# openxrlab/xrslam

Measured on AMD Instinct MI355X. Metric: frames/sec, full per-frame hot path (KLT tracker + sliding-window VI-BA), one sequence per GPU, higher is better.
Workload: dtype u8/i16 images, f32 LK with exact i64 reductions, f64 BA

## Files before the change

xrslam_amd/csrc/host/geometry.hpp:

```cpp
#pragma once
#include <array>
#include <cmath>
#include <map>
#include <numeric>
#include <random>
#include <vector>

#include "hla.hpp"

namespace xrh {

struct Intrinsics {
    double fx = 1, fy = 1, cx = 0, cy = 0;
};

inline V2 apply_k(V3 p, const Intrinsics &K) { return {p.x / p.z * K.fx + K.cx, p.y / p.z * K.fy + K.cy}; }
inline V3 remove_k(V2 p, const Intrinsics &K) { return normalized(V3{(p.x - K.cx) / K.fx, (p.y - K.cy) / K.fy, 1.0}); }

struct P34 {
    double m[12];
};
inline std::array<double, 4> triangulate_point(const std::vector<P34> &Ps, const std::vector<V3> &zs) {
    Dense A((int)zs.size() * 2, 4);
    for (size_t i = 0; i < zs.size(); ++i)
        for (int c = 0; c < 4; ++c) {
            A((int)i * 2, c) = zs[i].x * Ps[i].m[8 + c] - zs[i].z * Ps[i].m[c];
            A((int)i * 2 + 1, c) = zs[i].y * Ps[i].m[8 + c] - zs[i].z * Ps[i].m[4 + c];
        }
    std::vector<double> s;
    Dense V;
    jacobi_svd(A, s, V);
    return {V(0, 3), V(1, 3), V(2, 3), V(3, 3)};
}

class LotBox {
  public:
    explicit LotBox(size_t size) : cap_(0), lots_(size) { std::iota(lots_.begin(), lots_.end(), 0); }
    void seed(unsigned v) { engine_.seed(v); }
    void refill_all() { cap_ = 0; }
    size_t remaining() const { return lots_.size() - cap_; }
    size_t draw_without_replacement() {
        if (remaining() > 1) {
            std::uniform_int_distribution<size_t>::param_type pr(cap_, lots_.size() - 1);
            std::swap(lots_[cap_], lots_[dist_(engine_, pr)]);
            return lots_[cap_++];
        } else if (remaining() == 1) {
            cap_++;
            return lots_.back();
        }
        return size_t(-1);
    }

  private:
    size_t cap_;
    std::vector<size_t> lots_;
    std::default_random_engine engine_;
    std::uniform_int_distribution<size_t> dist_;
};

namespace fivept {

inline constexpr int pidx(int ex, int ey, int ez) { return ex * 16 + ey * 4 + ez; }
template <int D> struct Sup;
template <> struct Sup<1> {
    static constexpr int N = 4;
    static constexpr unsigned char idx[4] = {0, 1, 4, 16};
};
template <> struct Sup<2> {
    static constexpr int N = 10;
    static constexpr unsigned char idx[10] = {0, 1, 2, 4, 5, 8, 16, 17, 20, 32};
};
template <> struct Sup<3> {
    static constexpr int N = 20;
    static constexpr unsigned char idx[20] = {0, 1, 2, 3, 4, 5, 6, 8, 9, 12, 16, 17, 18, 20, 21, 24, 32, 33, 36, 48};
};
template <int D> inline constexpr int rank_of(int dense) {
    for (int k = 0; k < Sup<D>::N; ++k)
        if (Sup<D>::idx[k] == dense) return k;
    return -1;
}
template <int D> struct Poly {
    double c[Sup<D>::N];
    Poly() {
        for (double &v : c) v = 0.0;
    }
    double at(int ex, int ey, int ez) const { return c[rank_of<D>(pidx(ex, ey, ez))]; }
    double &at(int ex, int ey, int ez) { return c[rank_of<D>(pidx(ex, ey, ez))]; }
};
template <int D> inline Poly<D> padd(const Poly<D> &a, const Poly<D> &b, double sb = 1.0) {
    Poly<D> r;
    for (int k = 0; k < Sup<D>::N; ++k) r.c[k] = a.c[k] + sb * b.c[k];
    return r;
}
template <int D> inline Poly<D> pscale(const Poly<D> &a, double s) {
    Poly<D> r;
    for (int k = 0; k < Sup<D>::N; ++k) r.c[k] = a.c[k] * s;
    return r;
}
template <int DA, int DB> struct MulTable {
    unsigned char t[Sup<DA>::N][Sup<DB>::N];
    constexpr MulTable() : t() {
        for (int p = 0; p < Sup<DA>::N; ++p)
            for (int q = 0; q < Sup<DB>::N; ++q) t[p][q] = (unsigned char)rank_of<DA + DB>(Sup<DA>::idx[p] + Sup<DB>::idx[q]);
    }
};
template <int DA, int DB> inline Poly<DA + DB> pmul(const Poly<DA> &a, const Poly<DB> &b) {
    static constexpr MulTable<DA, DB> T{};
    Poly<DA + DB> r;
    for (int p = 0; p < Sup<DA>::N; ++p) {
        const double av = a.c[p];
        if (av == 0.0) continue;
        for (int q = 0; q < Sup<DB>::N; ++q) {
            const double bv = b.c[q];
            if (bv == 0.0) continue;
            r.c[T.t[p][q]] += av * bv;
        }
    }
    return r;
}

static constexpr int MONO[20][3] = {{3, 0, 0}, {2, 1, 0}, {1, 2, 0}, {0, 3, 0}, {2, 0, 1}, {1, 1, 1}, {0, 2, 1},
                                {1, 0, 2}, {0, 1, 2}, {0, 0, 3}, {2, 0, 0}, {1, 1, 0}, {0, 2, 0}, {1, 0, 1},
                                {0, 1, 1}, {0, 0, 2}, {1, 0, 0}, {0, 1, 0}, {0, 0, 1}, {0, 0, 0}};
enum { XXX = 0, XXY, XYY, YYY, XXZ, XYZ, YYZ, XZZ, YZZ, ZZZ, XX, XY, YY, XZ, YZ, ZZ, X, Y, Z, I };
struct MonoRank {
    unsigned char r[20];
    constexpr MonoRank() : r() {
        for (int m = 0; m < 20; ++m) r[m] = (unsigned char)rank_of<3>(pidx(MONO[m][0], MONO[m][1], MONO[m][2]));
    }
};

}

inline std::vector<M3> solve_essential_5pt(const std::array<V2, 5> &p1, const std::array<V2, 5> &p2) {
    using namespace fivept;
    for (int i = 0; i < 5; ++i)
        if (!std::isfinite(p1[i].x) || !std::isfinite(p1[i].y) || !std::isfinite(p2[i].x) || !std::isfinite(p2[i].y)) return {};
    Dense A(5, 9);
    for (int i = 0; i < 5; ++i) {
        const double h1[3] = {p1[i].x, p1[i].y, 1.0}, h2[3] = {p2[i].x, p2[i].y, 1.0};
        for (int j = 0; j < 3; ++j)
            for (int k = 0; k < 3; ++k) A(i, j * 3 + k) = h1[j] * h2[k];
    }
    std::vector<double> sv;
    Dense V;
    jacobi_svd(A, sv, V);
    double B[4][3][3];
    for (int b = 0; b < 4; ++b)
        for (int col = 0; col < 3; ++col)
            for (int row = 0; row < 3; ++row) B[b][row][col] = V(col * 3 + row, 5 + b);
    Poly<1> E[3][3];
    for (int i = 0; i < 3; ++i)
        for (int j = 0; j < 3; ++j) {
            E[i][j].at(1, 0, 0) = B[0][i][j];
            E[i][j].at(0, 1, 0) = B[1][i][j];
            E[i][j].at(0, 0, 1) = B[2][i][j];
            E[i][j].at(0, 0, 0) = B[3][i][j];
        }
    Poly<2> EEt[3][3];
    for (int i = 0; i < 3; ++i)
        for (int j = 0; j < 3; ++j) {
            Poly<2> s;
            for (int k = 0; k < 3; ++k) s = padd(s, pmul(E[i][k], E[j][k]));
            EEt[i][j] = s;
        }
    const Poly<2> tr = padd(padd(EEt[0][0], EEt[1][1]), EEt[2][2]);
    const Poly<2> half_tr = pscale(tr, 0.5);
    Dense polys(10, 20);
    static constexpr MonoRank MR{};
    for (int i = 0; i < 3; ++i)
        for (int j = 0; j < 3; ++j) {
            Poly<3> s;
            for (int k = 0; k < 3; ++k) s = padd(s, pmul(EEt[i][k], E[k][j]));
            s = padd(s, pmul(half_tr, E[i][j]), -1.0);
            for (int m = 0; m < 20; ++m) polys(i * 3 + j, m) = s.c[MR.r[m]];
        }
    {
        auto minor = [&](int r0, int c0, int r1, int c1, int r2, int c2, int r3, int c3) {
            return padd(pmul(E[r0][c0], E[r1][c1]), pmul(E[r2][c2], E[r3][c3]), -1.0);
        };
        const Poly<3> d = padd(padd(pmul(E[0][0], minor(1, 1, 2, 2, 1, 2, 2, 1)), pmul(E[0][1], minor(1, 0, 2, 2, 1, 2, 2, 0)), -1.0),
                               pmul(E[0][2], minor(1, 0, 2, 1, 1, 1, 2, 0)));
        for (int m = 0; m < 20; ++m) polys(9, m) = d.c[MR.r[m]];
    }
    std::array<int, 10> perm;
    for (int i = 0; i < 10; ++i) perm[i] = i;
    for (int i = 0; i < 10; ++i) {
        for (int j = i + 1; j < 10; ++j)
            if (std::fabs(polys(perm[i], i)) < std::fabs(polys(perm[j], i))) std::swap(perm[i], perm[j]);
        if (polys(perm[i], i) == 0) continue;
        const double d = polys(perm[i], i);
        for (int c = 0; c < 20; ++c) polys(perm[i], c) /= d;
        for (int j = i + 1; j < 10; ++j) {
            const double f = polys(perm[j], i);
            for (int c = 0; c < 20; ++c) polys(perm[j], c) -= polys(perm[i], c) * f;
        }
    }
    for (int i = 9; i > 0; --i)
        for (int j = 0; j < i; ++j) {
            const double f = polys(perm[j], i);
            for (int c = 0; c < 20; ++c) polys(perm[j], c) -= polys(perm[i], c) * f;
        }
    Dense action(10, 10);
    const int rows[6] = {XXX, XXY, XYY, XXZ, XYZ, XZZ};
    for (int r = 0; r < 6; ++r)
        for (int c = 0; c < 10; ++c) action(r, c) = -polys(perm[rows[r]], XX + c);
    action(6, XX - XX) = 1.0;
    action(7, XY - XX) = 1.0;
    action(8, XZ - XX) = 1.0;
    action(9, X - XX) = 1.0;
    std::vector<double> wr, wi;
    std::vector<std::vector<double>> vecs;
    real_eigen(action, wr, wi, vecs);
    std::vector<M3> out;
    for (int e = 0; e < 10; ++e) {
        if (vecs[e].empty()) continue;
        const std::vector<double> &h = vecs[e];
        const double w = h[I - XX];
        const double xs = h[X - XX] / w, ys = h[Y - XX] / w, zs = h[Z - XX] / w;
        M3 Em;
        for (int i = 0; i < 3; ++i)
            for (int j = 0; j < 3; ++j) Em(i, j) = B[0][i][j] * xs + B[1][i][j] * ys + B[2][i][j] * zs + B[3][i][j];
        out.push_back(Em);
    }
    return out;
}

inline double essential_geometric_error(const M3 &E, V2 p1, V2 p2) {
    V3 Ep1 = E * V3{p1.x, p1.y, 1.0};
    double r = p2.x * Ep1.x + p2.y * Ep1.y + Ep1.z;
    return r * r / (Ep1.x * Ep1.x + Ep1.y * Ep1.y);
}

inline M3 solve_rotation_2pt(const std::array<V3, 2> &a, const std::array<V3, 2> &b) {
    Dense cov(3, 3);
    for (int k = 0; k < 2; ++k)
        for (int i = 0; i < 3; ++i)
            for (int j = 0; j < 3; ++j) cov(i, j) += a[k][i] * b[k][j];
    for (double &v : cov.a) v *= 0.5;
    std::vector<double> s;
    Dense V, U;
    jacobi_svd(cov, s, V, &U);
    V3 u0{U(0, 0), U(1, 0), U(2, 0)}, u1{U(0, 1), U(1, 1), U(2, 1)}, u2{U(0, 2), U(1, 2), U(2, 2)};
    if (!(s[2] > 1e-12 * std::max(s[0], 1e-300))) {
        u2 = normalized(cross(u0, u1));
    }
    M3 Um, Vm;
    for (int i = 0; i < 3; ++i) {
        Um(i, 0) = u0[i];
        Um(i, 1) = u1[i];
        Um(i, 2) = u2[i];
        for (int j = 0; j < 3; ++j) Vm(i, j) = V(i, j);
    }
    M3 D = M3::identity();
    D(2, 2) = det(Vm * transpose(Um)) >= 0.0 ? 1.0 : -1.0;
    return Vm * D * transpose(Um);
}

template <size_t DoF, class Sample1, class Sample2, class Solver, class Evaluator>
M3 ransac_solve(const std::vector<Sample1> &d1, const std::vector<Sample2> &d2, double threshold, double confidence,
                size_t max_iteration, int seed, Solver solver, Evaluator make_eval, std::vector<char> &inlier_mask) {
    const size_t size = d1.size();
    LotBox lotbox(size);
    lotbox.seed((unsigned)seed);
    const double K = std::log(std::max(1 - confidence, 1.0e-5));
    size_t inlier_count = 0;
    M3 model;
    if (size < DoF) {
        inlier_mask.assign(size, 0);
        return model;
    }
    size_t iter_max = max_iteration;
    std::vector<char> cur_mask;
    for (size_t iter = 0; iter < iter_max; ++iter) {
        std::array<Sample1, DoF> s1;
        std::array<Sample2, DoF> s2;
        lotbox.refill_all();
        for (size_t si = 0; si < DoF; ++si) {
            size_t idx = lotbox.draw_without_replacement();
            s1[si] = d1[idx];
            s2[si] = d2[idx];
        }
        std::vector<M3> models = solver(s1, s2);
        for (const M3 &cur : models) {
            if (inlier_count == size) break;
            size_t cur_count = 0;
            cur_mask.assign(size, 0);
            auto eval = make_eval(cur);
            for (size_t i = 0; i < size; ++i) {
                double err = eval(d1[i], d2[i]);
                if (err <= threshold) {
                    cur_count++;
                    cur_mask[i] = 1;
                }
            }
            if (cur_count > inlier_count) {
                model = cur;
                inlier_count = cur_count;
                inlier_mask.swap(cur_mask);
                double ratio = inlier_count / (double)size;
                double N = K / std::log(1 - std::pow(ratio, 5));
                if (N < (double)iter_max) iter_max = (size_t)std::ceil(N);
            }
        }
    }
    return model;
}

inline M3 find_essential_matrix(const std::vector<V2> &p1, const std::vector<V2> &p2, std::vector<char> &mask,
                                double threshold = 1.0, double confidence = 0.999, size_t max_iteration = 1000,
                                int seed = 0) {
    mask.clear();
    auto solver = [](const std::array<V2, 5> &a, const std::array<V2, 5> &b) { return solve_essential_5pt(a, b); };
    auto make_eval = [](const M3 &E) {
        M3 Et = transpose(E);
        return [E, Et](V2 a, V2 b) { return essential_geometric_error(E, a, b) + essential_geometric_error(Et, b, a); };
    };
    return ransac_solve<5>(p1, p2, 2.0 * 3.84 * threshold * threshold, confidence, max_iteration, seed, solver,
                           make_eval, mask);
}

inline M3 find_rotation_matrix(const std::vector<V3> &p1, const std::vector<V3> &p2, std::vector<char> &mask,
                               double threshold, double confidence = 0.999, size_t max_iteration = 1000,
                               int seed = 0) {
    mask.clear();
    auto solver = [](const std::array<V3, 2> &a, const std::array<V3, 2> &b) {
        return std::vector<M3>{solve_rotation_2pt(a, b)};
    };
    auto make_eval = [](const M3 &R) { return [R](V3 a, V3 b) { return std::acos(dot(R * a, b)); }; };
    return ransac_solve<2>(p1, p2, 5.99 * threshold * threshold, confidence, max_iteration, seed, solver, make_eval,
                           mask);
}

}
```

xrslam_amd/csrc/host/hla.hpp:

```cpp
#pragma once
#include <algorithm>
#include <array>
#include <cmath>
#include <limits>
#include <vector>

namespace xrh {

struct V2 {
    double x = 0, y = 0;
};
struct V3 {
    double x = 0, y = 0, z = 0;
    double &operator[](int i) { return i == 0 ? x : (i == 1 ? y : z); }
    double operator[](int i) const { return i == 0 ? x : (i == 1 ? y : z); }
};
inline V3 operator+(V3 a, V3 b) { return {a.x + b.x, a.y + b.y, a.z + b.z}; }
inline V3 operator-(V3 a, V3 b) { return {a.x - b.x, a.y - b.y, a.z - b.z}; }
inline V3 operator-(V3 a) { return {-a.x, -a.y, -a.z}; }
inline V3 operator*(V3 a, double s) { return {a.x * s, a.y * s, a.z * s}; }
inline V3 operator*(double s, V3 a) { return a * s; }
inline V3 operator/(V3 a, double s) { return {a.x / s, a.y / s, a.z / s}; }
inline double dot(V3 a, V3 b) { return a.x * b.x + a.y * b.y + a.z * b.z; }
inline V3 cross(V3 a, V3 b) { return {a.y * b.z - a.z * b.y, a.z * b.x - a.x * b.z, a.x * b.y - a.y * b.x}; }
// ... 98 lines not shown
    for (int i = 0; i < m * n; ++i) fro2 += A[i] * A[i];
    const double null2 = 1e-30 * fro2;
    constexpr int NC = NT ? NT : 1;
    double st_norm[NC];
    bool st_ok[NC];
    std::vector<double> heap_norm;
    std::vector<char> heap_ok;
    double *norm2 = st_norm;
    bool *have = st_ok;
    if (!NT) {
        heap_norm.resize(n);
        heap_ok.resize(n);
        norm2 = heap_norm.data();
        have = reinterpret_cast<bool *>(heap_ok.data());
    }
    for (int j = 0; j < n; ++j) have[j] = false;
    auto col_norm2 = [&](int j) {
        if (!have[j]) {
            double t = 0;
            for (int i = 0; i < m; ++i) t += A[i * n + j] * A[i * n + j];
            norm2[j] = t;
            have[j] = true;
        }
        return norm2[j];
    };
    for (int sweep = 0; sweep < 60; ++sweep) {
        bool rotated = false;
        for (int p = 0; p < n - 1; ++p)
            for (int q = p + 1; q < n; ++q) {
                const double al = col_norm2(p), be = col_norm2(q);
                double ga = 0;
                for (int i = 0; i < m; ++i) ga += A[i * n + p] * A[i * n + q];
                if (ga == 0.0 || std::fabs(ga) <= 1e-16 * std::sqrt(al * be) || std::min(al, be) <= null2) continue;
                rotated = true;
                double zeta = (be - al) / (2.0 * ga);
                double t = 1.0 / (std::fabs(zeta) + std::sqrt(1.0 + zeta * zeta));
                if (zeta < 0) t = -t;
                double cs = 1.0 / std::sqrt(1.0 + t * t), sn = cs * t;
                for (int i = 0; i < m; ++i) {
                    double x = A[i * n + p], y = A[i * n + q];
                    A[i * n + p] = cs * x - sn * y;
                    A[i * n + q] = sn * x + cs * y;
                }
                have[p] = have[q] = false;
                for (int i = 0; i < n; ++i) {
                    double x = V[i * n + p], y = V[i * n + q];
                    V[i * n + p] = cs * x - sn * y;
                    V[i * n + q] = sn * x + cs * y;
                }
            }
        if (!rotated) break;
    }
}
inline void jacobi_svd(const Dense &A_in, std::vector<double> &s, Dense &V, Dense *U = nullptr) {
    const int m = A_in.r, n = A_in.c;
    Dense A = A_in;
    V = Dense(n, n);
    for (int i = 0; i < n; ++i) V(i, i) = 1.0;
    if (m == 5 && n == 9) jacobi_sweeps<5, 9>(A.a.data(), V.a.data(), m, n);
    else if (m == 3 && n == 3) jacobi_sweeps<3, 3>(A.a.data(), V.a.data(), m, n);
    else jacobi_sweeps<0, 0>(A.a.data(), V.a.data(), m, n);
    std::vector<double> nrm(n);
    std::vector<int> idx(n);
    for (int j = 0; j < n; ++j) {
        double t = 0;
        for (int i = 0; i < m; ++i) t += A(i, j) * A(i, j);
        nrm[j] = std::sqrt(t);
        idx[j] = j;
    }
    std::stable_sort(idx.begin(), idx.end(), [&](int a, int b) { return nrm[a] > nrm[b]; });
    Dense Vs(n, n);
    s.resize(n);
    if (U) *U = Dense(m, n);
    for (int j = 0; j < n; ++j) {
        s[j] = nrm[idx[j]];
        for (int i = 0; i < n; ++i) Vs(i, j) = V(i, idx[j]);
        if (U)
            for (int i = 0; i < m; ++i) (*U)(i, j) = s[j] > 0 ? A(i, idx[j]) / s[j] : 0.0;
    }
    V = Vs;
}

template <int NT>
inline void real_eigen_core(const double *Mbuf, int n_rt, std::vector<double> &wr, std::vector<double> &wi,
                            std::vector<std::vector<double>> &vecs) {
    const int n = NT ? NT : n_rt;
    double st_a[NT ? NT * NT : 1], st_b[NT ? NT * NT : 1], st_v[NT ? NT : 1];
    int st_piv[NT ? NT : 1];
    std::vector<double> heap_d;
    std::vector<int> heap_i;
    double *abuf = st_a, *bbuf = st_b, *v = st_v;
    int *piv = st_piv;
    if (!NT) {
        heap_d.resize((size_t)2 * n * n + n);
        heap_i.resize(n);
        abuf = heap_d.data();
        bbuf = abuf + (size_t)n * n;
        v = bbuf + (size_t)n * n;
        piv = heap_i.data();
    }
    for (int k = 0; k < n * n; ++k) abuf[k] = Mbuf[k];
    auto a = [=](int i, int j) -> double & { return abuf[i * n + j]; };
    auto B = [=](int i, int j) -> double & { return bbuf[i * n + j]; };
    auto M = [=](int i, int j) -> double { return Mbuf[i * n + j]; };
    for (int k = 0; k < n * n; ++k)
        if (!std::isfinite(Mbuf[k])) {
            wr.assign(n, std::numeric_limits<double>::quiet_NaN());
            wi.assign(n, std::numeric_limits<double>::quiet_NaN());
            vecs.assign(n, std::vector<double>());
            return;
        }
    for (int m = 1; m < n - 1; ++m) {
        double x = 0.0;
        int i = m;
        for (int j = m; j < n; ++j)
            if (std::fabs(a(j, m - 1)) > std::fabs(x)) {
                x = a(j, m - 1);
                i = j;
            }
        if (i != m) {
            for (int j = m - 1; j < n; ++j) std::swap(a(i, j), a(m, j));
            for (int j = 0; j < n; ++j) std::swap(a(j, i), a(j, m));
        }
        if (x != 0.0)
            for (i = m + 1; i < n; ++i) {
                double y = a(i, m - 1);
                if (y != 0.0) {
                    y /= x;
                    a(i, m - 1) = y;
                    for (int j = m; j < n; ++j) a(i, j) -= y * a(m, j);
                    for (int j = 0; j < n; ++j) a(j, m) += y * a(j, i);
                }
            }
    }
    for (int i = 2; i < n; ++i)
        for (int j = 0; j < i - 1; ++j) a(i, j) = 0.0;
    wr.assign(n, 0.0);
    wi.assign(n, 0.0);
    int nn = n - 1, its = 0;
    double t = 0.0, p = 0, q = 0, r = 0, s = 0, w = 0, x = 0, y = 0, z = 0;
    double anorm = 0.0;
    for (int i = 0; i < n; ++i)
        for (int j = std::max(i - 1, 0); j < n; ++j) anorm += std::fabs(a(i, j));
    while (nn >= 0) {
        its = 0;
        int l;
        do {
            for (l = nn; l >= 1; --l) {
                s = std::fabs(a(l - 1, l - 1)) + std::fabs(a(l, l));
                if (s == 0.0) s = anorm;
                if (std::fabs(a(l, l - 1)) + s == s) {
                    a(l, l - 1) = 0.0;
                    break;
                }
            }
            x = a(nn, nn);
            if (l == nn) {
                wr[nn] = x + t;
                wi[nn--] = 0.0;
            } else {
                y = a(nn - 1, nn - 1);
                w = a(nn, nn - 1) * a(nn - 1, nn);
                if (l == nn - 1) {
                    p = 0.5 * (y - x);
                    q = p * p + w;
                    z = std::sqrt(std::fabs(q));
                    x += t;
                    if (q >= 0.0) {
                        z = p + (p >= 0 ? std::fabs(z) : -std::fabs(z));
                        wr[nn - 1] = wr[nn] = x + z;
                        if (z != 0.0) wr[nn] = x - w / z;
                        wi[nn - 1] = wi[nn] = 0.0;
                    } else {
                        wr[nn - 1] = wr[nn] = x + p;
                        wi[nn - 1] = -(wi[nn] = z);
                    }
                    nn -= 2;
                } else {
                    if (its == 60) return;
                    if (its == 10 || its == 20) {
                        t += x;
                        for (int i = 0; i <= nn; ++i) a(i, i) -= x;
                        s = std::fabs(a(nn, nn - 1)) + std::fabs(a(nn - 1, nn - 2));
                        y = x = 0.75 * s;
                        w = -0.4375 * s * s;
                    }
                    ++its;
                    int m;
                    for (m = nn - 2; m >= l; --m) {
                        z = a(m, m);
                        r = x - z;
                        s = y - z;
                        p = (r * s - w) / a(m + 1, m) + a(m, m + 1);
                        q = a(m + 1, m + 1) - z - r - s;
                        r = a(m + 2, m + 1);
                        s = std::fabs(p) + std::fabs(q) + std::fabs(r);
                        p /= s;
                        q /= s;
                        r /= s;
                        if (m == l) break;
                        double u = std::fabs(a(m, m - 1)) * (std::fabs(q) + std::fabs(r));
                        double v = std::fabs(p) * (std::fabs(a(m - 1, m - 1)) + std::fabs(z) + std::fabs(a(m + 1, m + 1)));
                        if (u + v == v) break;
                    }
                    for (int i = m + 2; i <= nn; ++i) {
                        a(i, i - 2) = 0.0;
                        if (i != m + 2) a(i, i - 3) = 0.0;
                    }
                    for (int k = m; k <= nn - 1; ++k) {
                        if (k != m) {
                            p = a(k, k - 1);
                            q = a(k + 1, k - 1);
                            r = 0.0;
                            if (k != nn - 1) r = a(k + 2, k - 1);
                            if ((x = std::fabs(p) + std::fabs(q) + std::fabs(r)) != 0.0) {
                                p /= x;
                                q /= x;
                                r /= x;
                            }
                        }
                        double sg = std::sqrt(p * p + q * q + r * r);
                        s = p >= 0 ? sg : -sg;
                        if (s != 0.0) {
                            if (k == m) {
                                if (l != m) a(k, k - 1) = -a(k, k - 1);
                            } else {
                                a(k, k - 1) = -s * x;
                            }
                            p += s;
                            x = p / s;
                            y = q / s;
                            z = r / s;
                            q /= p;
                            r /= p;
                            for (int j = k; j <= nn; ++j) {
                                p = a(k, j) + q * a(k + 1, j);
                                if (k != nn - 1) {
                                    p += r * a(k + 2, j);
                                    a(k + 2, j) -= p * z;
                                }
                                a(k + 1, j) -= p * y;
                                a(k, j) -= p * x;
                            }
                            int mmin = nn < k + 3 ? nn : k + 3;
                            for (int i = l; i <= mmin; ++i) {
                                p = x * a(i, k) + y * a(i, k + 1);
                                if (k != nn - 1) {
                                    p += z * a(i, k + 2);
                                    a(i, k + 2) -= p * r;
                                }
                                a(i, k + 1) -= p * q;
                                a(i, k) -= p;
                            }
                        }
                    }
                }
            }
        } while (l < nn - 1);
    }
    vecs.assign(n, std::vector<double>());
    for (int e = 0; e < n; ++e) {
        if (std::fabs(wi[e]) >= 1.0e-10) continue;
        const double lam = wr[e];
        double scale = 0;
        for (int i = 0; i < n; ++i)
            for (int j = 0; j < n; ++j) {
                B(i, j) = M(i, j) - (i == j ? lam : 0.0);
                scale = std::max(scale, std::fabs(M(i, j)));
            }
        const double eps = std::max(scale, 1.0) * 1e-13;
        for (int i = 0; i < n; ++i) B(i, i) += eps * (1 + i % 3);
        for (int k = 0; k < n; ++k) {
            int pk = k;
            for (int i = k + 1; i < n; ++i)
                if (std::fabs(B(i, k)) > std::fabs(B(pk, k))) pk = i;
            piv[k] = pk;
            if (pk != k)
                for (int j = 0; j < n; ++j) std::swap(B(k, j), B(pk, j));
            if (B(k, k) == 0.0) B(k, k) = eps;
            for (int i = k + 1; i < n; ++i) {
                B(i, k) /= B(k, k);
                for (int j = k + 1; j < n; ++j) B(i, j) -= B(i, k) * B(k, j);
            }
        }
        for (int k = 0; k < n; ++k) v[k] = 1.0;
        for (int it = 0; it < 4; ++it) {
            for (int k = 0; k < n; ++k) {
                if (piv[k] != k) std::swap(v[k], v[piv[k]]);
                for (int i = k + 1; i < n; ++i) v[i] -= B(i, k) * v[k];
            }
            for (int i = n - 1; i >= 0; --i) {
                for (int j = i + 1; j < n; ++j) v[i] -= B(i, j) * v[j];
                v[i] /= B(i, i);
            }
            double nrm = 0;
            for (int k = 0; k < n; ++k) nrm += v[k] * v[k];
            nrm = std::sqrt(nrm);
            if (!(nrm > 0) || !std::isfinite(nrm)) break;
            for (int k = 0; k < n; ++k) v[k] /= nrm;
        }
        vecs[e].assign(v, v + n);
    }
}
inline void real_eigen(const Dense &M, std::vector<double> &wr, std::vector<double> &wi,
                       std::vector<std::vector<double>> &vecs) {
    if (M.r == 10) real_eigen_core<10>(M.a.data(), M.r, wr, wi, vecs);
    else real_eigen_core<0>(M.a.data(), M.r, wr, wi, vecs);
}

}
```

xrslam_amd/csrc/host/pipeline.hpp:

```cpp
#pragma once
#include <chrono>
#include <climits>
#include <algorithm>
#include <cstdio>
#include <cstring>
#include <atomic>
#include <condition_variable>
#include <deque>
#include <exception>
#include <functional>
#include <mutex>
#include <optional>
#include <stdexcept>
#include <thread>
#include <tuple>
#include <unordered_map>
#include <unordered_set>

#include "../host_select.hpp"
#include "../hostprof.hpp"
#include "ba_dump.hpp"
#include "config.hpp"
#include "covariance.hpp"
#include "map.hpp"
// ... 92 lines not shown
        }
    }

  private:
    enum { IDLE = 0, POSTED, DONE, QUIT };
    static void relax() {
#if defined(__x86_64__) || defined(__i386__)
        __builtin_ia32_pause();
#else
        std::this_thread::yield();
#endif
    }
    template <class Pred> void await(Pred pred, long spin_us) {
        const auto t0 = std::chrono::steady_clock::now();
        for (;;) {
            for (int spin = 0; spin < 256; ++spin) {
                if (pred()) return;
                relax();
            }
            if (std::chrono::steady_clock::now() - t0 > std::chrono::microseconds(spin_us)) break;
        }
        std::unique_lock<std::mutex> lk(m_);
        cv_.wait(lk, pred);
    }
    void loop() {
        if (device_ >= 0) xrhip_bind_device(device_);
        for (;;) {
            await([this] {
                const int s = state_.load(std::memory_order_acquire);
                return s == POSTED || s == QUIT;
            }, 2000);
            if (state_.load(std::memory_order_acquire) == QUIT) return;
            try {
                job_();
            } catch (...) {
                error_ = std::current_exception();
            }
            state_.store(DONE, std::memory_order_release);
            {
                std::lock_guard<std::mutex> lk(m_);
            }
            cv_.notify_all();
        }
    }
    int device_;
    std::function<void()> job_;
    std::exception_ptr error_;
    std::atomic<int> state_{IDLE};
    std::mutex m_;
    std::condition_variable cv_;
    std::thread th_;
};

struct Pipeline {
    Config config;
    xrhip_klt *klt = nullptr;
    xrhip_ba *ba = nullptr;
    xrhip_ba *ba_marg = nullptr;
    xrhip_ba *ba_aux = nullptr;
    xrhip_ba *ba_ft = nullptr;
    xrhip_ba *ba_sub = nullptr;
    std::mutex pool_mutex;
    std::unique_ptr<JobThread> marg_launcher;
    bool marg_launch_pending = false;
    void marg_launch_wait() {
        if (!marg_launch_pending) return;
        marg_launch_pending = false;
        marg_launcher->wait();
    }
    IdSource ids;
    std::vector<xrhip_image *> image_pool;
    double noise36[36];
    StageTimes times;
    struct Covariance {
        bool enabled = false;
        double t = 0.0;
        double state[225] = {0.0};
        int status = -1;
        double rcond = 0.0;
        std::vector<std::pair<long long, double>> landmark_var;
        std::string error;
    } cov;
    unsigned long ba_generation = 0;
    bool undistort_on_device = false;
    void set_device_undistort(const char *model) {
        if (!model || !*model) {
            hip_check(xrhip_klt_set_undistort_map(klt, nullptr), "xrhip_klt_set_undistort_map");
            undistort_on_device = false;
            return;
        }
        const double K4[4] = {config.K.fx, config.K.fy, config.K.cx, config.K.cy};
        const std::vector<uint32_t> map = build_undistort_map((int)config.cam_resolution[0], (int)config.cam_resolution[1], K4,
                                                              config.cam_distortion, 4, model);
        hip_check(xrhip_klt_set_undistort_map(klt, map.data()), "xrhip_klt_set_undistort_map");
        undistort_on_device = true;
    }
    SwtLogger swt_log;
    SyncLogger sync_log;
    BaDumper ba_dump;
    InitLogger init_log;
    OutLogger out_log;

    static bool check_lk_params(const Config &c, xrhip_lk_params &p) {
        auto whole = [](double v, double lo, double hi) { return v >= lo && v <= hi && v == (double)(long long)v; };
        const double win = c.feature_tracker_lk_window_size, lev = c.feature_tracker_lk_max_level, cnt = c.feature_tracker_lk_max_iterations,
                     eps = c.feature_tracker_lk_epsilon;
        char b[256];
// ... 295 lines not shown
                  "xrhip_ba_preintegrate_begin");
        return ok;
    }
    std::vector<double> batch_collect(xrhip_ba *ctx, size_t n_jobs) {
        std::vector<double> out((size_t)XRHIP_IMU_DIM * n_jobs);
        WallTimer wt_w_preintegrate(preintegrate_slot(ctx));
        hip_check(xrhip_ba_preintegrate_end(ctx, out.data()), "xrhip_ba_preintegrate_end");
        return out;
    }
    std::vector<PreInt *> pending_pre_;
};

inline HipImage::~HipImage() {
    if (h && owner) owner->recycle_image(h);
    h = nullptr;
}
inline void HipImage::release_image_buffer() {
    if (h && owner) owner->recycle_image(h);
    h = nullptr;
}

inline void predict(const PreInt &pre, const Frame *o, Frame *n) {
    const V3 gravity{0, 0, -9.80665};
    const double dt = pre.dt();
    n->motion.bg = o->motion.bg;
    n->motion.ba = o->motion.ba;
    n->motion.v = o->motion.v + gravity * dt + o->pose.q * pre.dv();
    n->pose.p = o->pose.p + 0.5 * gravity * dt * dt + o->motion.v * dt + o->pose.q * pre.dp();
    n->pose.q = o->pose.q * pre.dq();
}

inline void frame_detect_keypoints(Pipeline &P, Frame *f) {
    WallTimer sc_t(P.times.scope[SC_FT_DETECT]);
    const Config &c = P.config;
    std::vector<double> existing(2 * f->keypoint_num());
    for (size_t i = 0; i < f->keypoint_num(); ++i) {
        V2 px = apply_k(f->bearings[i], f->K);
        existing[2 * i] = px.x;
        existing[2 * i + 1] = px.y;
    }
    const int maxp = (int)c.feature_tracker_max_keypoint_detection;
    std::vector<double> fresh(2 * (size_t)std::max(maxp, 1));
    int n_new = 0;
    WallTimer wt_w_detect(P.times.w_detect);
    hip_check(xrhip_image_detect(f->image->h, existing.data(), (int)f->keypoint_num(), maxp,
                                 c.feature_tracker_min_keypoint_distance, fresh.data(), &n_new),
              "xrhip_image_detect");
    for (int i = 0; i < n_new; ++i) f->append_keypoint(remove_k(V2{fresh[2 * i], fresh[2 * i + 1]}, f->K));
}

inline void frame_track_keypoints(Pipeline &P, Frame *cur, Frame *next, std::function<void(Frame *)> *deferred_tag = nullptr) {
    WallTimer sc_t(P.times.scope[SC_FT_TRACK]);
    const Config &c = P.config;
    const size_t n = cur->keypoint_num();
    std::vector<double> curr_px(2 * n), next_px(2 * n);
    for (size_t i = 0; i < n; ++i) {
        V2 px = apply_k(cur->bearings[i], cur->K);
        curr_px[2 * i] = px.x;
        curr_px[2 * i + 1] = px.y;
    }
    int has_guess = 0;
    if (c.feature_tracker_predict_keypoints) {
        Quat dq = (cur->camera.q_cs.conjugate() * cur->imu.q_cs * next->preintegration.dq() *
                   next->imu.q_cs.conjugate() * next->camera.q_cs)
                      .conjugate();
        for (size_t i = 0; i < n; ++i) {
            V2 px = apply_k(dq * cur->bearings[i], next->K);
            next_px[2 * i] = px.x;
            next_px[2 * i + 1] = px.y;
        }
        has_guess = 1;
    }
    std::vector<uint8_t> st8(std::max<size_t>(n, 1), 0);
    {
        WallTimer wt_w_track(P.times.w_track);
        hip_check(xrhip_image_track(cur->image->h, next->image->h, curr_px.data(), next_px.data(), has_guess,
                                    st8.data(), (int)n),
                  "xrhip_image_track");
    }
    xrhip::HostProfScope hp_post(4, "ft_track: after LK (all)");
    std::optional<xrhip::HostProfScope> hp_a(std::in_place, 5, "ft_track: bearings");
    std::vector<char> status(st8.begin(), st8.begin() + n), mask;
    std::vector<V2> cur_h, next_h;
    std::vector<V3> next_bearings;
    cur_h.reserve(n);
    next_h.reserve(n);
    next_bearings.reserve(n);
    for (size_t i = 0; i < n; ++i) {
        const V3 &b = cur->bearings[i];
        cur_h.push_back({b.x / b.z, b.y / b.z});
        V3 nb = remove_k(V2{next_px[2 * i], next_px[2 * i + 1]}, next->K);
        next_h.push_back({nb.x / nb.z, nb.y / nb.z});
        next_bearings.push_back(nb);
    }
    hp_a.reset();
    {
        WallTimer sc_e(P.times.scope[SC_RANSAC_E]);
        find_essential_matrix(cur_h, next_h, mask, 1.0);
    }
    for (size_t i = 0; i < status.size() && i < mask.size(); ++i)
        if (!mask[i]) status[i] = 0;
    M3 R;
    {
        WallTimer sc_r(P.times.scope[SC_RANSAC_R]);
        R = find_rotation_matrix(cur->bearings, next_bearings, mask, (M_PI / 180.0) * c.rotation_ransac_threshold);
    }
    xrhip::HostProfScope hp_b(6, "ft_track: angles+poisson+append");
    std::optional<xrhip::HostProfScope> hp_c(std::in_place, 13, "ft_track: angles");
    {
        std::vector<std::pair<V3, V3>> pairs;
        pairs.reserve(mask.size());
        for (size_t i = 0; i < mask.size(); ++i)
            if (mask[i]) pairs.emplace_back(R * cur->bearings[i], next_bearings[i]);
        const double threshold = c.rotation_misalignment_threshold;
        auto decide = [pairs = std::move(pairs), threshold, next](Frame *copy) {
            std::vector<double> angles;
            angles.reserve(pairs.size());
            for (const auto &pr : pairs) angles.push_back(std::acos(dot(pr.first, pr.second)) * 180 / M_PI);
            std::sort(angles.begin(), angles.end());
            const double misalignment = angles.size() > 0 ? angles[angles.size() * 7 / 10] : 0;
            if (misalignment < threshold) {
                next->tag(FT_NO_TRANSLATION) = true;
                if (copy) copy->tag(FT_NO_TRANSLATION) = true;
            }
        };
        if (deferred_tag) *deferred_tag = std::move(decide);
        else decide(nullptr);
    }

    hp_c.emplace(14, "ft_track: by_length+poisson");
    std::vector<std::pair<size_t, size_t>> by_length;
    by_length.reserve(n);
    for (size_t i = 0; i < n; ++i) {
        if (status[i] == 0) continue;
        Track *t = cur->get_track(i);
        if (t == nullptr) continue;
        by_length.emplace_back(i, t->keypoint_num());
    }
    std::sort(by_length.begin(), by_length.end(), [](const auto &a, const auto &b) { return a.second > b.second; });
    xrhip::PoissonDisk2 filter(c.feature_tracker_min_keypoint_distance, (int)c.cam_resolution[0], (int)c.cam_resolution[1]);
    for (auto &[ki, len] : by_length) {
        (void)len;
        Track *t = cur->get_track(ki);
        if (filter.permit(next_px[2 * ki], next_px[2 * ki + 1]) && (!t || !t->tag(TT_TRASH))) {
            filter.preset(next_px[2 * ki], next_px[2 * ki + 1]);
        } else {
            status[ki] = 0;
        }
    }
    hp_c.reset();
    xrhip::HostProfScope hp_d(15, "ft_track: append");
    for (size_t i = 0; i < n; ++i) {
        if (status[i]) {
            size_t nk = next->keypoint_num();
            next->append_keypoint(next_bearings[i]);
            cur->get_track(i, nullptr)->add_keypoint(next, nk);
        }
    }
}

inline void resolve_marginalization(Pipeline &P, MargPrior *prior) {
    if (!prior || !prior->pending) return;
    P.marg_launch_wait();
    const size_t n = prior->frames.size(), R = 15 * n;
    std::vector<double> si(R * R), iv(R), lin(16 * n);
    {
        WallTimer wt_w_marginalize(P.times.w_marginalize);
        hip_check(xrhip_ba_marginalize_end(P.ba_marg, si.data(), iv.data(), lin.data()), "xrhip_ba_marginalize_end");
    }
    prior->sqrt_info.swap(si);
    prior->infovec.swap(iv);
    prior->lin.swap(lin);
    prior->pending = false;
}

class BaBuilder {
  public:
    explicit BaBuilder(Pipeline &P) : P_(P), gen_(++P.ba_generation) {
        obs_tgt_.reserve(2048);
        obs_ref_.reserve(2048);
        obs_lm_.reserve(2048);
        obs_zt_.reserve(3 * 2048);
        obs_zr_.reserve(3 * 2048);
        tracks_.reserve(512);
        lfix_.reserve(512);
    }
    int frame_index(Frame *f, bool as_parameter, bool with_motion = true) {
        if (f->ba_gen != gen_) {
            f->ba_gen = gen_;
            f->ba_index = (int)frames_.size();
            frames_.push_back(f);
            fix_.push_back(XRHIP_FIX_POSE | XRHIP_FIX_MOTION);
        }
// ... 2504 lines not shown
```

xrslam_amd/csrc/host_select.hpp:

```cpp
#pragma once
#include <cmath>
#include <cstdint>
#include <unordered_map>
#include <vector>

namespace xrhip {

class PoissonDisk2 {
  public:
    explicit PoissonDisk2(double radius, int width = 0, int height = 0)
        : r2_(radius * radius), cell_(radius / std::sqrt(2.0)), span_((int)std::ceil(std::sqrt(2.0))) {
        if (width > 0 && height > 0) {
            gw_ = (int)std::floor(width / cell_) + 1 + 2 * kMargin;
            gh_ = (int)std::floor(height / cell_) + 1 + 2 * kMargin;
            dense_.assign((size_t)gw_ * gh_, -1);
        }
    }

    void preset(double x, double y) {
        slot(ix(x), ix(y)) = (int)pts_.size() / 2;
        pts_.push_back(x);
        pts_.push_back(y);
    }

    bool permit(double x, double y) const {
        const int cx = ix(x), cy = ix(y);
        const int bx = cx - span_, by = cy - span_, ex = cx + span_, ey = cy + span_;
        if (inside(bx, by) && inside(ex, ey + 1)) {
            for (int yy = by; yy <= ey + 1; ++yy) {
                const int x0 = yy == by ? bx + 1 : bx, x1 = yy == ey + 1 ? bx : ex;
                const int *row = dense_.data() + (size_t)(yy + kMargin) * gw_ + kMargin;
                for (int xx = x0; xx <= x1; ++xx) {
                    const int at = row[xx];
                    if (at >= 0) {
                        const double dx = x - pts_[2 * at], dy = y - pts_[2 * at + 1];
                        if (dx * dx + dy * dy < r2_) return false;
                    }
                }
            }
            return true;
        }
        int x_it = bx, y_it = by;
        while (y_it <= ey) {
            ++x_it;
            if (x_it > ex) {
                x_it = bx;
                ++y_it;
            }
            const int at = lookup(x_it, y_it);
            if (at >= 0) {
                const double dx = x - pts_[2 * at], dy = y - pts_[2 * at + 1];
                if (dx * dx + dy * dy < r2_) return false;
            }
        }
        return true;
    }

    bool insert(double x, double y) {
        if (!permit(x, y)) return false;
        preset(x, y);
        return true;
    }

  private:
    static constexpr int kMargin = 4;
    int ix(double v) const { return (int)std::floor(v / cell_); }
    static int64_t key(int a, int b) { return ((int64_t)a << 32) ^ (uint32_t)b; }
    bool inside(int a, int b) const { return a >= -kMargin && b >= -kMargin && a < gw_ - kMargin && b < gh_ - kMargin; }
    int lookup(int a, int b) const {
// ... 60 lines not shown
```

Measured before the change: 1720.

## Remove heap allocations from host RANSAC and frame-tracking hot path

Replaces the Dense/vector temporaries in the 5-point essential solver, the 2-point rotation solver and the eigen solver with fixed-size stack buffers, using a templated Jacobi SVD. RANSAC now reuses per-pipeline scratch (lotbox, masks, model list), evaluates residuals in blocks, and stops scoring a model once it can no longer beat the best inlier count. Frame tracking keeps its vectors and the Poisson-disk filter in a persistent scratch struct instead of reallocating them every frame. The deferred tag closure now points at shared scratch, so it must run before the next frame overwrites that state.

```diff
diff --git a/xrslam_amd/csrc/host/geometry.hpp b/xrslam_amd/csrc/host/geometry.hpp
--- a/xrslam_amd/csrc/host/geometry.hpp
+++ b/xrslam_amd/csrc/host/geometry.hpp
@@ -35,7 +35,13 @@
 
 class LotBox {
   public:
+    LotBox() : cap_(0) {}
     explicit LotBox(size_t size) : cap_(0), lots_(size) { std::iota(lots_.begin(), lots_.end(), 0); }
+    void reset(size_t size) {
+        cap_ = 0;
+        lots_.resize(size);
+        std::iota(lots_.begin(), lots_.end(), 0);
+    }
     void seed(unsigned v) { engine_.seed(v); }
     void refill_all() { cap_ = 0; }
     size_t remaining() const { return lots_.size() - cap_; }
@@ -132,19 +138,20 @@
 
 }
 
-inline std::vector<M3> solve_essential_5pt(const std::array<V2, 5> &p1, const std::array<V2, 5> &p2) {
+constexpr int kMaxEssential = 10;
+inline int solve_essential_5pt_into(const std::array<V2, 5> &p1, const std::array<V2, 5> &p2, M3 *out) {
     using namespace fivept;
     for (int i = 0; i < 5; ++i)
-        if (!std::isfinite(p1[i].x) || !std::isfinite(p1[i].y) || !std::isfinite(p2[i].x) || !std::isfinite(p2[i].y)) return {};
-    Dense A(5, 9);
+        if (!std::isfinite(p1[i].x) || !std::isfinite(p1[i].y) || !std::isfinite(p2[i].x) || !std::isfinite(p2[i].y)) return 0;
+    double A[5 * 9];
     for (int i = 0; i < 5; ++i) {
         const double h1[3] = {p1[i].x, p1[i].y, 1.0}, h2[3] = {p2[i].x, p2[i].y, 1.0};
         for (int j = 0; j < 3; ++j)
-            for (int k = 0; k < 3; ++k) A(i, j * 3 + k) = h1[j] * h2[k];
-    }
-    std::vector<double> sv;
-    Dense V;
-    jacobi_svd(A, sv, V);
+            for (int k = 0; k < 3; ++k) A[i * 9 + j * 3 + k] = h1[j] * h2[k];
+    }
+    double sv[9], Vbuf[9 * 9];
+    jacobi_svd_fixed<5, 9>(A, sv, Vbuf);
+    auto V = [&](int i, int j) { return Vbuf[i * 9 + j]; };
     double B[4][3][3];
     for (int b = 0; b < 4; ++b)
         for (int col = 0; col < 3; ++col)
@@ -166,7 +173,8 @@
         }
     const Poly<2> tr = padd(padd(EEt[0][0], EEt[1][1]), EEt[2][2]);
     const Poly<2> half_tr = pscale(tr, 0.5);
-    Dense polys(10, 20);
+    double polys_buf[10 * 20];
+    auto polys = [&](int i, int j) -> double & { return polys_buf[i * 20 + j]; };
     static constexpr MonoRank MR{};
     for (int i = 0; i < 3; ++i)
         for (int j = 0; j < 3; ++j) {
@@ -201,7 +209,9 @@
             const double f = polys(perm[j], i);
             for (int c = 0; c < 20; ++c) polys(perm[j], c) -= polys(perm[i], c) * f;
         }
-    Dense action(10, 10);
+    double action_buf[10 * 10];
+    for (double &v : action_buf) v = 0.0;
+    auto action = [&](int i, int j) -> double & { return action_buf[i * 10 + j]; };
     const int rows[6] = {XXX, XXY, XYY, XXZ, XYZ, XZZ};
     for (int r = 0; r < 6; ++r)
         for (int c = 0; c < 10; ++c) action(r, c) = -polys(perm[rows[r]], XX + c);
@@ -209,21 +219,26 @@
     action(7, XY - XX) = 1.0;
     action(8, XZ - XX) = 1.0;
     action(9, X - XX) = 1.0;
-    std::vector<double> wr, wi;
-    std::vector<std::vector<double>> vecs;
-    real_eigen(action, wr, wi, vecs);
-    std::vector<M3> out;
+    double wr[10], wi[10], vecs[10 * 10];
+    char has[10];
+    real_eigen_core<10>(action_buf, 10, wr, wi, vecs, has);
+    int n_out = 0;
     for (int e = 0; e < 10; ++e) {
-        if (vecs[e].empty()) continue;
-        const std::vector<double> &h = vecs[e];
+        if (!has[e]) continue;
+        const double *h = vecs + e * 10;
         const double w = h[I - XX];
         const double xs = h[X - XX] / w, ys = h[Y - XX] / w, zs = h[Z - XX] / w;
         M3 Em;
         for (int i = 0; i < 3; ++i)
             for (int j = 0; j < 3; ++j) Em(i, j) = B[0][i][j] * xs + B[1][i][j] * ys + B[2][i][j] * zs + B[3][i][j];
-        out.push_back(Em);
-    }
-    return out;
+        out[n_out++] = Em;
+    }
+    return n_out;
+}
+inline std::vector<M3> solve_essential_5pt(const std::array<V2, 5> &p1, const std::array<V2, 5> &p2) {
+    M3 Es[kMaxEssential];
+    const int n = solve_essential_5pt_into(p1, p2, Es);
+    return std::vector<M3>(Es, Es + n);
 }
 
 inline double essential_geometric_error(const M3 &E, V2 p1, V2 p2) {
@@ -233,14 +248,15 @@
 }
 
 inline M3 solve_rotation_2pt(const std::array<V3, 2> &a, const std::array<V3, 2> &b) {
-    Dense cov(3, 3);
+    double cov[9] = {0, 0, 0, 0, 0, 0, 0, 0, 0};
     for (int k = 0; k < 2; ++k)
         for (int i = 0; i < 3; ++i)
-            for (int j = 0; j < 3; ++j) cov(i, j) += a[k][i] * b[k][j];
-    for (double &v : cov.a) v *= 0.5;
-    std::vector<double> s;
-    Dense V, U;
-    jacobi_svd(cov, s, V, &U);
+            for (int j = 0; j < 3; ++j) cov[i * 3 + j] += a[k][i] * b[k][j];
+    for (double &v : cov) v *= 0.5;
+    double s[3], Vb[9], Ub[9];
+    jacobi_svd_fixed<3, 3>(cov, s, Vb, Ub);
+    auto V = [&](int i, int j) { return Vb[i * 3 + j]; };
+    auto U = [&](int i, int j) { return Ub[i * 3 + j]; };
     V3 u0{U(0, 0), U(1, 0), U(2, 0)}, u1{U(0, 1), U(1, 1), U(2, 1)}, u2{U(0, 2), U(1, 2), U(2, 2)};
     if (!(s[2] > 1e-12 * std::max(s[0], 1e-300))) {
         u2 = normalized(cross(u0, u1));
@@ -257,22 +273,36 @@
     return Vm * D * transpose(Um);
 }
 
+
+struct RansacScratch {
+    LotBox lotbox;
+    std::vector<char> cur_mask;
+    std::vector<M3> models;
+    size_t iterations = 0;
+};
+
+constexpr size_t kRansacBlock = 32;
 template <size_t DoF, class Sample1, class Sample2, class Solver, class Evaluator>
-M3 ransac_solve(const std::vector<Sample1> &d1, const std::vector<Sample2> &d2, double threshold, double confidence,
-                size_t max_iteration, int seed, Solver solver, Evaluator make_eval, std::vector<char> &inlier_mask) {
+M3 ransac_solve_scratch(const std::vector<Sample1> &d1, const std::vector<Sample2> &d2, double threshold, double confidence,
+                        size_t max_iteration, int seed, Solver solver, Evaluator make_eval, std::vector<char> &inlier_mask,
+                        RansacScratch &sc) {
     const size_t size = d1.size();
-    LotBox lotbox(size);
+    LotBox &lotbox = sc.lotbox;
+    lotbox.reset(size);
     lotbox.seed((unsigned)seed);
     const double K = std::log(std::max(1 - confidence, 1.0e-5));
     size_t inlier_count = 0;
     M3 model;
+    sc.iterations = 0;
     if (size < DoF) {
         inlier_mask.assign(size, 0);
         return model;
     }
     size_t iter_max = max_iteration;
-    std::vector<char> cur_mask;
+    std::vector<char> &cur_mask = sc.cur_mask;
+    double err[kRansacBlock];
     for (size_t iter = 0; iter < iter_max; ++iter) {
+        sc.iterations = iter + 1;
         std::array<Sample1, DoF> s1;
         std::array<Sample2, DoF> s2;
         lotbox.refill_all();
@@ -281,20 +311,25 @@
             s1[si] = d1[idx];
             s2[si] = d2[idx];
         }
-        std::vector<M3> models = solver(s1, s2);
-        for (const M3 &cur : models) {
+        sc.models.clear();
+        solver(s1, s2, sc.models);
+        for (const M3 &cur : sc.models) {
             if (inlier_count == size) break;
             size_t cur_count = 0;
-            cur_mask.assign(size, 0);
+            cur_mask.resize(size);
             auto eval = make_eval(cur);
-            for (size_t i = 0; i < size; ++i) {
-                double err = eval(d1[i], d2[i]);
-                if (err <= threshold) {
-                    cur_count++;
-                    cur_mask[i] = 1;
+            bool beaten = false;
+            for (size_t i0 = 0; i0 < size && !beaten; i0 += kRansacBlock) {
+                const size_t cnt = std::min(kRansacBlock, size - i0);
+                eval(&d1[i0], &d2[i0], cnt, err);
+                for (size_t k = 0; k < cnt; ++k) {
+                    const char in = err[k] <= threshold ? 1 : 0;
+                    cur_mask[i0 + k] = in;
+                    cur_count += (size_t)in;
                 }
+                beaten = cur_count + (size - i0 - cnt) <= inlier_count;
             }
-            if (cur_count > inlier_count) {
+            if (!beaten) {
                 model = cur;
                 inlier_count = cur_count;
                 inlier_mask.swap(cur_mask);
@@ -307,29 +342,54 @@
     return model;
 }
 
+template <size_t DoF, class Sample1, class Sample2, class Solver, class Evaluator>
+M3 ransac_solve(const std::vector<Sample1> &d1, const std::vector<Sample2> &d2, double threshold, double confidence,
+                size_t max_iteration, int seed, Solver solver, Evaluator make_eval, std::vector<char> &inlier_mask) {
+    RansacScratch sc;
+    auto solve_into = [&](const std::array<Sample1, DoF> &a, const std::array<Sample2, DoF> &b, std::vector<M3> &out) {
+        for (const M3 &m : solver(a, b)) out.push_back(m);
+    };
+    auto make_block_eval = [&](const M3 &m) {
+        return [pt = make_eval(m)](const Sample1 *a, const Sample2 *b, size_t cnt, double *err) {
+            for (size_t k = 0; k < cnt; ++k) err[k] = pt(a[k], b[k]);
+        };
+    };
+    return ransac_solve_scratch<DoF>(d1, d2, threshold, confidence, max_iteration, seed, solve_into, make_block_eval, inlier_mask, sc);
+}
+
 inline M3 find_essential_matrix(const std::vector<V2> &p1, const std::vector<V2> &p2, std::vector<char> &mask,
                                 double threshold = 1.0, double confidence = 0.999, size_t max_iteration = 1000,
-                                int seed = 0) {
+                                int seed = 0, RansacScratch *scratch = nullptr) {
     mask.clear();
-    auto solver = [](const std::array<V2, 5> &a, const std::array<V2, 5> &b) { return solve_essential_5pt(a, b); };
+    auto solver = [](const std::array<V2, 5> &a, const std::array<V2, 5> &b, std::vector<M3> &out) {
+        M3 Es[kMaxEssential];
+        const int n = solve_essential_5pt_into(a, b, Es);
+        out.insert(out.end(), Es, Es + n);
+    };
     auto make_eval = [](const M3 &E) {
         M3 Et = transpose(E);
-        return [E, Et](V2 a, V2 b) { return essential_geometric_error(E, a, b) + essential_geometric_error(Et, b, a); };
-    };
-    return ransac_solve<5>(p1, p2, 2.0 * 3.84 * threshold * threshold, confidence, max_iteration, seed, solver,
-                           make_eval, mask);
+        return [E, Et](const V2 *a, const V2 *b, size_t cnt, double *err) {
+            for (size_t k = 0; k < cnt; ++k) err[k] = essential_geometric_error(E, a[k], b[k]) + essential_geometric_error(Et, b[k], a[k]);
+        };
+    };
+    RansacScratch local;
+    return ransac_solve_scratch<5>(p1, p2, 2.0 * 3.84 * threshold * threshold, confidence, max_iteration, seed, solver, make_eval, mask,
+                                   scratch ? *scratch : local);
 }
 
 inline M3 find_rotation_matrix(const std::vector<V3> &p1, const std::vector<V3> &p2, std::vector<char> &mask,
                                double threshold, double confidence = 0.999, size_t max_iteration = 1000,
-                               int seed = 0) {
+                               int seed = 0, RansacScratch *scratch = nullptr) {
     mask.clear();
-    auto solver = [](const std::array<V3, 2> &a, const std::array<V3, 2> &b) {
-        return std::vector<M3>{solve_rotation_2pt(a, b)};
-    };
-    auto make_eval = [](const M3 &R) { return [R](V3 a, V3 b) { return std::acos(dot(R * a, b)); }; };
-    return ransac_solve<2>(p1, p2, 5.99 * threshold * threshold, confidence, max_iteration, seed, solver, make_eval,
-                           mask);
-}
-
-}
+    auto solver = [](const std::array<V3, 2> &a, const std::array<V3, 2> &b, std::vector<M3> &out) { out.push_back(solve_rotation_2pt(a, b)); };
+    auto make_eval = [](const M3 &R) {
+        return [R](const V3 *a, const V3 *b, size_t cnt, double *err) {
+            for (size_t k = 0; k < cnt; ++k) err[k] = std::acos(dot(R * a[k], b[k]));
+        };
+    };
+    RansacScratch local;
+    return ransac_solve_scratch<2>(p1, p2, 5.99 * threshold * threshold, confidence, max_iteration, seed, solver, make_eval, mask,
+                                   scratch ? *scratch : local);
+}
+
+}
diff --git a/xrslam_amd/csrc/host/hla.hpp b/xrslam_amd/csrc/host/hla.hpp
--- a/xrslam_amd/csrc/host/hla.hpp
+++ b/xrslam_amd/csrc/host/hla.hpp
@@ -174,6 +174,28 @@
         if (!rotated) break;
     }
 }
+template <int M, int N> inline void jacobi_svd_fixed(double *A, double *s, double *V, double *U = nullptr) {
+    double Vr[N * N];
+    for (int i = 0; i < N * N; ++i) Vr[i] = 0.0;
+    for (int i = 0; i < N; ++i) Vr[i * N + i] = 1.0;
+    jacobi_sweeps<M, N>(A, Vr, M, N);
+    double nrm[N];
+    int idx[N];
+    for (int j = 0; j < N; ++j) {
+        double t = 0;
+        for (int i = 0; i < M; ++i) t += A[i * N + j] * A[i * N + j];
+        nrm[j] = std::sqrt(t);
+        int k = j;
+        for (; k > 0 && nrm[j] > nrm[idx[k - 1]]; --k) idx[k] = idx[k - 1];
+        idx[k] = j;
+    }
+    for (int j = 0; j < N; ++j) {
+        s[j] = nrm[idx[j]];
+        for (int i = 0; i < N; ++i) V[i * N + j] = Vr[i * N + idx[j]];
+        if (U)
+            for (int i = 0; i < M; ++i) U[i * N + j] = s[j] > 0 ? A[i * N + idx[j]] / s[j] : 0.0;
+    }
+}
 inline void jacobi_svd(const Dense &A_in, std::vector<double> &s, Dense &V, Dense *U = nullptr) {
     const int m = A_in.r, n = A_in.c;
     Dense A = A_in;
@@ -204,9 +226,9 @@
 }
 
 template <int NT>
-inline void real_eigen_core(const double *Mbuf, int n_rt, std::vector<double> &wr, std::vector<double> &wi,
-                            std::vector<std::vector<double>> &vecs) {
+inline bool real_eigen_core(const double *Mbuf, int n_rt, double *wr, double *wi, double *vecs, char *has) {
     const int n = NT ? NT : n_rt;
+    for (int e = 0; e < n; ++e) has[e] = 0;
     double st_a[NT ? NT * NT : 1], st_b[NT ? NT * NT : 1], st_v[NT ? NT : 1];
     int st_piv[NT ? NT : 1];
     std::vector<double> heap_d;
@@ -227,10 +249,8 @@
     auto M = [=](int i, int j) -> double { return Mbuf[i * n + j]; };
     for (int k = 0; k < n * n; ++k)
         if (!std::isfinite(Mbuf[k])) {
-            wr.assign(n, std::numeric_limits<double>::quiet_NaN());
-            wi.assign(n, std::numeric_limits<double>::quiet_NaN());
-            vecs.assign(n, std::vector<double>());
-            return;
+            for (int e = 0; e < n; ++e) wr[e] = wi[e] = std::numeric_limits<double>::quiet_NaN();
+            return true;
         }
     for (int m = 1; m < n - 1; ++m) {
         double x = 0.0;
@@ -257,8 +277,7 @@
     }
     for (int i = 2; i < n; ++i)
         for (int j = 0; j < i - 1; ++j) a(i, j) = 0.0;
-    wr.assign(n, 0.0);
-    wi.assign(n, 0.0);
+    for (int e = 0; e < n; ++e) wr[e] = wi[e] = 0.0;
     int nn = n - 1, its = 0;
     double t = 0.0, p = 0, q = 0, r = 0, s = 0, w = 0, x = 0, y = 0, z = 0;
     double anorm = 0.0;
@@ -299,7 +318,7 @@
                     }
                     nn -= 2;
                 } else {
-                    if (its == 60) return;
+                    if (its == 60) return false;
                     if (its == 10 || its == 20) {
                         t += x;
                         for (int i = 0; i <= nn; ++i) a(i, i) -= x;
@@ -380,17 +399,15 @@
             }
         } while (l < nn - 1);
     }
-    vecs.assign(n, std::vector<double>());
+    double scale = 0;
+    for (int i = 0; i < n; ++i)
+        for (int j = 0; j < n; ++j) scale = std::max(scale, std::fabs(M(i, j)));
+    const double eps = std::max(scale, 1.0) * 1e-13;
     for (int e = 0; e < n; ++e) {
         if (std::fabs(wi[e]) >= 1.0e-10) continue;
         const double lam = wr[e];
-        double scale = 0;
         for (int i = 0; i < n; ++i)
-            for (int j = 0; j < n; ++j) {
-                B(i, j) = M(i, j) - (i == j ? lam : 0.0);
-                scale = std::max(scale, std::fabs(M(i, j)));
-            }
-        const double eps = std::max(scale, 1.0) * 1e-13;
+            for (int j = 0; j < n; ++j) B(i, j) = M(i, j) - (i == j ? lam : 0.0);
         for (int i = 0; i < n; ++i) B(i, i) += eps * (1 + i % 3);
         for (int k = 0; k < n; ++k) {
             int pk = k;
@@ -421,13 +438,24 @@
             if (!(nrm > 0) || !std::isfinite(nrm)) break;
             for (int k = 0; k < n; ++k) v[k] /= nrm;
         }
-        vecs[e].assign(v, v + n);
-    }
+        for (int k = 0; k < n; ++k) vecs[e * n + k] = v[k];
+        has[e] = 1;
+    }
+    return true;
 }
 inline void real_eigen(const Dense &M, std::vector<double> &wr, std::vector<double> &wi,
                        std::vector<std::vector<double>> &vecs) {
-    if (M.r == 10) real_eigen_core<10>(M.a.data(), M.r, wr, wi, vecs);
-    else real_eigen_core<0>(M.a.data(), M.r, wr, wi, vecs);
-}
-
-}
+    const int n = M.r;
+    std::vector<double> flat((size_t)n * n);
+    std::vector<char> has(n);
+    wr.resize(n);
+    wi.resize(n);
+    const bool done = n == 10 ? real_eigen_core<10>(M.a.data(), n, wr.data(), wi.data(), flat.data(), has.data())
+                              : real_eigen_core<0>(M.a.data(), n, wr.data(), wi.data(), flat.data(), has.data());
+    if (!done) return;
+    vecs.assign(n, std::vector<double>());
+    for (int e = 0; e < n; ++e)
+        if (has[e]) vecs[e].assign(flat.begin() + (size_t)e * n, flat.begin() + (size_t)(e + 1) * n);
+}
+
+}
diff --git a/xrslam_amd/csrc/host/pipeline.hpp b/xrslam_amd/csrc/host/pipeline.hpp
--- a/xrslam_amd/csrc/host/pipeline.hpp
+++ b/xrslam_amd/csrc/host/pipeline.hpp
@@ -168,7 +168,24 @@
     std::thread th_;
 };
 
+struct FtScratch {
+    std::vector<double> curr_px, next_px, angles;
+    std::vector<uint8_t> st8;
+    std::vector<char> status, mask;
+    std::vector<V2> cur_h, next_h;
+    std::vector<V3> next_bearings;
+    std::vector<std::pair<V3, V3>> pairs;
+    std::vector<std::pair<size_t, size_t>> by_length;
+    RansacScratch ransac_e, ransac_r;
+    std::optional<xrhip::PoissonDisk2> filter;
+    double filter_radius = 0.0;
+    int filter_w = 0, filter_h = 0;
+    double tag_threshold = 0.0;
+    Frame *tag_next = nullptr;
+};
+
 struct Pipeline {
+    FtScratch ft;
     Config config;
     xrhip_klt *klt = nullptr;
     xrhip_ba *ba = nullptr;
@@ -570,8 +587,11 @@
 inline void frame_track_keypoints(Pipeline &P, Frame *cur, Frame *next, std::function<void(Frame *)> *deferred_tag = nullptr) {
     WallTimer sc_t(P.times.scope[SC_FT_TRACK]);
     const Config &c = P.config;
+    FtScratch &S = P.ft;
     const size_t n = cur->keypoint_num();
-    std::vector<double> curr_px(2 * n), next_px(2 * n);
+    std::vector<double> &curr_px = S.curr_px, &next_px = S.next_px;
+    curr_px.resize(2 * n);
+    next_px.assign(2 * n, 0.0);
     for (size_t i = 0; i < n; ++i) {
         V2 px = apply_k(cur->bearings[i], cur->K);
         curr_px[2 * i] = px.x;
@@ -589,7 +609,8 @@
         }
         has_guess = 1;
     }
-    std::vector<uint8_t> st8(std::max<size_t>(n, 1), 0);
+    std::vector<uint8_t> &st8 = S.st8;
+    st8.assign(std::max<size_t>(n, 1), 0);
     {
         WallTimer wt_w_track(P.times.w_track);
         hip_check(xrhip_image_track(cur->image->h, next->image->h, curr_px.data(), next_px.data(), has_guess,
@@ -598,57 +619,58 @@
     }
     xrhip::HostProfScope hp_post(4, "ft_track: after LK (all)");
     std::optional<xrhip::HostProfScope> hp_a(std::in_place, 5, "ft_track: bearings");
-    std::vector<char> status(st8.begin(), st8.begin() + n), mask;
-    std::vector<V2> cur_h, next_h;
-    std::vector<V3> next_bearings;
-    cur_h.reserve(n);
-    next_h.reserve(n);
-    next_bearings.reserve(n);
+    std::vector<char> &status = S.status, &mask = S.mask;
+    status.assign(st8.begin(), st8.begin() + n);
+    std::vector<V2> &cur_h = S.cur_h, &next_h = S.next_h;
+    std::vector<V3> &next_bearings = S.next_bearings;
+    cur_h.resize(n);
+    next_h.resize(n);
+    next_bearings.resize(n);
     for (size_t i = 0; i < n; ++i) {
         const V3 &b = cur->bearings[i];
-        cur_h.push_back({b.x / b.z, b.y / b.z});
+        cur_h[i] = {b.x / b.z, b.y / b.z};
         V3 nb = remove_k(V2{next_px[2 * i], next_px[2 * i + 1]}, next->K);
-        next_h.push_back({nb.x / nb.z, nb.y / nb.z});
-        next_bearings.push_back(nb);
+        next_h[i] = {nb.x / nb.z, nb.y / nb.z};
+        next_bearings[i] = nb;
     }
     hp_a.reset();
     {
         WallTimer sc_e(P.times.scope[SC_RANSAC_E]);
-        find_essential_matrix(cur_h, next_h, mask, 1.0);
+        find_essential_matrix(cur_h, next_h, mask, 1.0, 0.999, 1000, 0, &S.ransac_e);
     }
     for (size_t i = 0; i < status.size() && i < mask.size(); ++i)
         if (!mask[i]) status[i] = 0;
     M3 R;
     {
         WallTimer sc_r(P.times.scope[SC_RANSAC_R]);
-        R = find_rotation_matrix(cur->bearings, next_bearings, mask, (M_PI / 180.0) * c.rotation_ransac_threshold);
+        R = find_rotation_matrix(cur->bearings, next_bearings, mask, (M_PI / 180.0) * c.rotation_ransac_threshold, 0.999, 1000, 0, &S.ransac_r);
     }
     xrhip::HostProfScope hp_b(6, "ft_track: angles+poisson+append");
     std::optional<xrhip::HostProfScope> hp_c(std::in_place, 13, "ft_track: angles");
     {
-        std::vector<std::pair<V3, V3>> pairs;
-        pairs.reserve(mask.size());
+        S.pairs.clear();
         for (size_t i = 0; i < mask.size(); ++i)
-            if (mask[i]) pairs.emplace_back(R * cur->bearings[i], next_bearings[i]);
-        const double threshold = c.rotation_misalignment_threshold;
-        auto decide = [pairs = std::move(pairs), threshold, next](Frame *copy) {
-            std::vector<double> angles;
-            angles.reserve(pairs.size());
-            for (const auto &pr : pairs) angles.push_back(std::acos(dot(pr.first, pr.second)) * 180 / M_PI);
+            if (mask[i]) S.pairs.emplace_back(R * cur->bearings[i], next_bearings[i]);
+        S.tag_threshold = c.rotation_misalignment_threshold;
+        S.tag_next = next;
+        auto decide = [sp = &S](Frame *copy) {
+            std::vector<double> &angles = sp->angles;
+            angles.clear();
+            for (const auto &pr : sp->pairs) angles.push_back(std::acos(dot(pr.first, pr.second)) * 180 / M_PI);
             std::sort(angles.begin(), angles.end());
             const double misalignment = angles.size() > 0 ? angles[angles.size() * 7 / 10] : 0;
-            if (misalignment < threshold) {
-                next->tag(FT_NO_TRANSLATION) = true;
+            if (misalignment < sp->tag_threshold) {
+                sp->tag_next->tag(FT_NO_TRANSLATION) = true;
                 if (copy) copy->tag(FT_NO_TRANSLATION) = true;
             }
         };
-        if (deferred_tag) *deferred_tag = std::move(decide);
+        if (deferred_tag) *deferred_tag = decide;
         else decide(nullptr);
     }
 
     hp_c.emplace(14, "ft_track: by_length+poisson");
-    std::vector<std::pair<size_t, size_t>> by_length;
-    by_length.reserve(n);
+    std::vector<std::pair<size_t, size_t>> &by_length = S.by_length;
+    by_length.clear();
     for (size_t i = 0; i < n; ++i) {
         if (status[i] == 0) continue;
         Track *t = cur->get_track(i);
@@ -656,7 +678,16 @@
         by_length.emplace_back(i, t->keypoint_num());
     }
     std::sort(by_length.begin(), by_length.end(), [](const auto &a, const auto &b) { return a.second > b.second; });
-    xrhip::PoissonDisk2 filter(c.feature_tracker_min_keypoint_distance, (int)c.cam_resolution[0], (int)c.cam_resolution[1]);
+    const int fw = (int)c.cam_resolution[0], fh = (int)c.cam_resolution[1];
+    if (S.filter && S.filter_radius == c.feature_tracker_min_keypoint_distance && S.filter_w == fw && S.filter_h == fh) {
+        S.filter->reset();
+    } else {
+        S.filter.emplace(c.feature_tracker_min_keypoint_distance, fw, fh);
+        S.filter_radius = c.feature_tracker_min_keypoint_distance;
+        S.filter_w = fw;
+        S.filter_h = fh;
+    }
+    xrhip::PoissonDisk2 &filter = *S.filter;
     for (auto &[ki, len] : by_length) {
         (void)len;
         Track *t = cur->get_track(ki);
diff --git a/xrslam_amd/csrc/host_select.hpp b/xrslam_amd/csrc/host_select.hpp
--- a/xrslam_amd/csrc/host_select.hpp
+++ b/xrslam_amd/csrc/host_select.hpp
@@ -1,4 +1,5 @@
 #pragma once
+#include <algorithm>
 #include <cmath>
 #include <cstdint>
 #include <unordered_map>
@@ -15,6 +16,12 @@
             gh_ = (int)std::floor(height / cell_) + 1 + 2 * kMargin;
             dense_.assign((size_t)gw_ * gh_, -1);
         }
+    }
+
+    void reset() {
+        pts_.clear();
+        std::fill(dense_.begin(), dense_.end(), -1);
+        sparse_.clear();
     }
 
     void preset(double x, double y) {
```

After: 1643. -4.5%, worse.
